# ribal-aladeeb/reinforcement-learning-2048

Measured on AMD Instinct MI355X. Metric: 2048 env steps/sec + DQN updates/sec at 64k parallel boards, 1→8 MI355X, higher is better.
Workload: dtype u8

## Files before the change

### reinforcement-learning-2048_amd/csrc/g2048_learn64.hip

```cpp
#include <hip/hip_runtime.h>
#include <math.h>
#include <stdint.h>
#include <stdlib.h>

#include "../../include/g2048.h"
#include "g2048_board.hpp"
#include "g2048_common.hpp"

namespace {

constexpr int NT = 256;
constexpr int S = 64;
constexpr int XS = 17;
constexpr int HS = 65;
constexpr int P_W1 = 0, P_B1 = 1024, P_W2 = 1088, P_B2 = 1344, P_N = 1348;
constexpr int SLAB = P_N + 4;
constexpr int MAX_SLABS = 256;

struct Net64 {
    double *w1, *b1, *w2, *b2;
};

struct alignas(16) Smem {
    double x[S * XS];
    double h[S * HS];
    double w2[2][4 * 64];
    double b1[2][64];
    double b2[2][4];
    double qa[S * 4];
    double qb[S * 4];
    double y[S];
    double dq[S];
    double loss[S];
    int act[S];
};

__device__ __forceinline__ int64_t sample_row(int64_t b, unsigned long long ep,
                                              unsigned long long count, uint32_t lo, uint32_t hi) {
    const uint4 u = g2048::philox10(
        make_uint4((uint32_t)b, (uint32_t)((uint64_t)b >> 32), (uint32_t)ep,
                   (uint32_t)(ep >> 32) | (g2048::DOMAIN_SAMPLE << 30)),
        lo, hi);
    return (int64_t)__umul64hi(((unsigned long long)u.y << 32) | u.x, count);
}

__device__ __forceinline__ void put_row(double* xr, uint4 v) {
    const uint32_t w[4] = {v.x, v.y, v.z, v.w};
#pragma unroll
    for (int k = 0; k < 4; ++k) {
        xr[4 * k + 0] = (double)(w[k] & 0xFFu);
        xr[4 * k + 1] = (double)((w[k] >> 8) & 0xFFu);
        xr[4 * k + 2] = (double)((w[k] >> 16) & 0xFFu);
        xr[4 * k + 3] = (double)(w[k] >> 24);
    }
}

__device__ __forceinline__ void forward(Smem& M, const double (&w1r)[16], int net, double* q) {
    const int t = threadIdx.x, j = t & 63, rq = t >> 6;
    const double bj = M.b1[net][j];
#pragma unroll 4
    for (int rr = 0; rr < 16; ++rr) {
        const int s = rq * 16 + rr;
        const double* xr = M.x + s * XS;
        double acc = 0.0;
#pragma unroll
        for (int k = 0; k < 16; ++k) acc = fma(w1r[k], xr[k], acc);
        const double pre = acc + bj;
        M.h[s * HS + j] = pre > 0.0 ? pre : 0.0;
    }
    __syncthreads();
    const int s = t >> 2, a = t & 3;
    const double* hr = M.h + s * HS;
    const double* w2 = M.w2[net] + a * 64;
    double acc = 0.0;
#pragma unroll 8
    for (int jj = 0; jj < 64; ++jj) acc = fma(w2[jj], hr[jj], acc);
    q[s * 4 + a] = acc + M.b2[net][a];
    __syncthreads();
}

struct UpdArgs64 {
    Net64 on, tg;
    const uint4 *s, *s2;
    const uint8_t *a, *d;
    const int32_t* r;
    const unsigned long long* count;
    const unsigned long long* step;
    const int64_t* idx_in;
    int64_t batch;
    uint32_t seed_lo, seed_hi;
    float gamma;
    int double_dqn;
    int64_t* idx_out;
    double* y_out;
    double* slab;
    unsigned long long* step_next;
};

typedef uint32_t u32x2 __attribute__((ext_vector_type(2)));
constexpr int AUX_SC1 = 16;
__device__ __forceinline__ __amdgpu_buffer_rsrc_t slab_rsrc(const double* base) {
    return __builtin_amdgcn_make_buffer_rsrc(const_cast<double*>(base), 0, 0x7FFFFFFF, 0x00020000);
}
template <bool COH>
__device__ __forceinline__ void slab_put(double* sl, int e, double v) {
    if constexpr (COH)
        __builtin_amdgcn_raw_buffer_store_b64(__builtin_bit_cast(u32x2, v), slab_rsrc(sl),
                                              (uint32_t)e * 8u, 0u, AUX_SC1);
    else
        sl[e] = v;
}

template <bool COH>
__device__ __forceinline__ void update_tiles64(const UpdArgs64& A) {
    __shared__ Smem M;
    const int t = threadIdx.x, j = t & 63, qd = t >> 6;
    const unsigned long long ep = A.idx_in ? 0ull : *A.step;
    const unsigned long long count = A.idx_in ? 0ull : *A.count;
    if (blockIdx.x == 0 && t == 0) *A.step_next = *A.step + 1ull;
    const Net64 nets[2] = {A.tg, A.on};
    double w1t[16], w1o[16];
#pragma unroll
    for (int k = 0; k < 16; ++k) {
        w1t[k] = A.tg.w1[j * 16 + k];
        w1o[k] = A.on.w1[j * 16 + k];
    }
    for (int i = t; i < 2 * 256; i += NT) M.w2[i >> 8][i & 255] = nets[i >> 8].w2[i & 255];
    if (t < 128) M.b1[t >> 6][t & 63] = nets[t >> 6].b1[t & 63];
    if (t < 8) M.b2[t >> 2][t & 3] = nets[t >> 2].b2[t & 3];
    double w2o[4];
#pragma unroll
    for (int a = 0; a < 4; ++a) w2o[a] = A.on.w2[a * 64 + j];
    double g_w1[4] = {0.0, 0.0, 0.0, 0.0}, g_b1 = 0.0, g_w2 = 0.0, g_b2 = 0.0, g_loss = 0.0;
    const int64_t ntiles = (A.batch + S - 1) / S;
    for (int64_t tile = blockIdx.x; tile < ntiles; tile += gridDim.x) {
        const int64_t b = tile * S + t;
        uint4 sv = make_uint4(0u, 0u, 0u, 0u);
        double rj = 0.0;
        float disc = 0.f;
        bool ok = false;
        __syncthreads();
        if (t < S) {
            uint4 s2v = make_uint4(0u, 0u, 0u, 0u);
            int aj = 0;
            ok = b < A.batch;
            if (ok) {
                const int64_t row =
                    A.idx_in ? A.idx_in[b] : sample_row(b, ep, count, A.seed_lo, A.seed_hi);
                A.idx_out[b] = row;
                s2v = A.s2[row];
                sv = A.s[row];
                aj = A.a[row];
                rj = (double)A.r[row];
                disc = (float)(1 - (int)A.d[row]) * A.gamma;
            }
            put_row(M.x + t * XS, s2v);
            M.act[t] = aj;
        }
        __syncthreads();
        forward(M, w1t, 0, M.qa);
        forward(M, w1o, 1, M.qb);
        if (t < S) {
            const double* qo = M.qb + t * 4;
            const double* qt = M.qa + t * 4;
            double next;
            if (A.double_dqn) {
                const uint32_t as = g2048::argmax4_torch(qo[0], qo[1], qo[2], qo[3]);
                next = qt[as];
            } else {
                next = g2048::qmax4_torch(qt[0], qt[1], qt[2], qt[3]);
            }
            double y;
            {
#pragma clang fp contract(off)
                y = rj + (double)disc * next;
            }
            M.y[t] = y;
            if (ok) A.y_out[b] = y;
            put_row(M.x + t * XS, sv);
        }
        __syncthreads();
        forward(M, w1o, 1, M.qb);
        if (t < S) {
            double dq = 0.0, l = 0.0;
            if (ok) {
#pragma clang fp contract(off)
                const double e = M.qb[t * 4 + M.act[t]] - M.y[t];
                dq = 2.0 * e;
                l = e * e;
            }
            M.dq[t] = dq;
            M.loss[t] = l;
        }
        __syncthreads();
        {
            double acc = 0.0, accb = 0.0;
            for (int s = 0; s < S; ++s) {
                if (M.act[s] == qd) {
                    acc = fma(M.dq[s], M.h[s * HS + j], acc);
                    accb += M.dq[s];
                }
            }
            g_w2 += acc;
            if (j == 0) g_b2 += accb;
        }
        if (t == 0) {
            double l = 0.0;
            for (int s = 0; s < S; ++s) l += M.loss[s];
            g_loss += l;
        }
        __syncthreads();
#pragma unroll 4
        for (int rr = 0; rr < 16; ++rr) {
            const int s = qd * 16 + rr;
            double& hv = M.h[s * HS + j];
            const double w = M.act[s] == 0 ? w2o[0] : M.act[s] == 1 ? w2o[1]
                           : M.act[s] == 2 ? w2o[2] : w2o[3];
            hv = hv > 0.0 ? M.dq[s] * w : 0.0;
        }
        __syncthreads();
        {
            double acc[4] = {0.0, 0.0, 0.0, 0.0}, accb = 0.0;
            for (int s = 0; s < S; ++s) {
                const double dh = M.h[s * HS + j];
                const double* xr = M.x + s * XS + 4 * qd;
#pragma unroll
                for (int i = 0; i < 4; ++i) acc[i] = fma(dh, xr[i], acc[i]);
                accb += dh;
            }
#pragma unroll
            for (int i = 0; i < 4; ++i) g_w1[i] += acc[i];
            if (qd == 0) g_b1 += accb;
        }
    }
    double* sl = A.slab + (int64_t)blockIdx.x * SLAB;
#pragma unroll
    for (int i = 0; i < 4; ++i) slab_put<COH>(sl, P_W1 + j * 16 + 4 * qd + i, g_w1[i]);
    if (qd == 0) slab_put<COH>(sl, P_B1 + j, g_b1);
    slab_put<COH>(sl, P_W2 + qd * 64 + j, g_w2);
    if (j == 0) slab_put<COH>(sl, P_B2 + qd, g_b2);
    if (t == 0) slab_put<COH>(sl, P_N, g_loss);
}

__global__ __launch_bounds__(NT) void k_dense64_update_f64(UpdArgs64 A) { update_tiles64<false>(A); }

constexpr int RW = 16;
static_assert(MAX_SLABS <= RW * 16, "reduction covers at most RW*16 slabs");

struct RedArgs64 {
    const double* slab;
    int nslab;
    double* grad;
    double* loss;
    const unsigned long long* step_next;
    unsigned long long* step;
    double* p[4];
    double* tp[4];
    unsigned long long sync_every;
    double* m;
    double* v;
    double lr, b1, b2, eps;
    int adam;
};

template <int NW, bool COH>
__device__ __forceinline__ void reduce_positions64(const RedArgs64& A, int chunk,
                                                   unsigned long long t, double (*part)[64]) {
    const int lane = threadIdx.x & 63, wave = threadIdx.x >> 6;
    const int pos = chunk * 64 + lane;
    const int k = pos < P_B1 ? 0 : pos < P_W2 ? 1 : pos < P_B2 ? 2 : 3;
    const int base[4] = {P_W1, P_B1, P_W2, P_B2};
    const bool adam = A.adam && wave == 0 && pos < P_N;
    double am = 0.0, av = 0.0, ap = 0.0;
    if (adam) {
        am = A.m[pos];
        av = A.v[pos];
        ap = A.p[k][pos - base[k]];
    }
    constexpr int PW = RW / NW;
    const bool okp = pos <= P_N;
    const int pc = okp ? pos : P_N;
    double v[PW][16];
#pragma unroll
    for (int i = 0; i < PW; ++i)
#pragma unroll
        for (int u = 0; u < 16; ++u) {
            const int g = wave + NW * i + RW * u;
            const bool ok = okp && g < A.nslab;
            const int64_t e = (int64_t)(g < A.nslab ? g : 0) * SLAB + pc;
            double x;
            if constexpr (COH)
                x = __builtin_bit_cast(double, __builtin_amdgcn_raw_buffer_load_b64(
                                                   slab_rsrc(A.slab), (uint32_t)(e * 8), 0u, AUX_SC1));
            else
                x = A.slab[e];
            v[i][u] = ok ? x : 0.0;
        }
#pragma unroll
    for (int i = 0; i < PW; ++i) {
        double r = 0.0;
#pragma unroll
        for (int u = 0; u < 16; ++u) r += v[i][u];
        part[wave + NW * i][lane] = r;
    }
    __syncthreads();
    if (wave == 0 && pos <= P_N) {
        double sum = part[0][lane];
        for (int j = 1; j < RW; ++j) sum += part[j][lane];
        if (pos == P_N) {
            if (A.loss) *A.loss = sum;
        } else {
            if (A.grad) A.grad[pos] = sum;
            if (adam) {
                const double np = g2048::adam64((double)t, A.lr, A.b1, A.b2, A.eps, sum, am, av, ap);
                A.m[pos] = am;
                A.v[pos] = av;
                A.p[k][pos - base[k]] = np;
                if (A.sync_every && t % A.sync_every == 0ull) A.tp[k][pos - base[k]] = np;
            }
        }
    }
}

constexpr int RCHUNKS = (P_N + 1 + 63) / 64;

__global__ __launch_bounds__(64 * RW) void k_dense64_reduce_f64(RedArgs64 A) {
    __shared__ double part[RW][64];
    reduce_positions64<RW, false>(A, blockIdx.x, A.adam ? *A.step_next : 0ull, part);
    if (A.step && blockIdx.x == 0 && threadIdx.x == 0) *A.step = *A.step_next;
}

struct Upd1Args64 {
    UpdArgs64 U;
    RedArgs64 R;
    unsigned int* arrive;
};

__global__ __launch_bounds__(NT) void k_dense64_update1_f64(Upd1Args64 A) {
    const unsigned long long t_next = *A.U.step + 1ull;
    update_tiles64<true>(A.U);
    __shared__ unsigned int s_arrival;
    __shared__ double part[RW][64];
    const unsigned grid = gridDim.x;
    __builtin_amdgcn_s_waitcnt(0);
    __syncthreads();
    if (threadIdx.x == 0)
        s_arrival = __hip_atomic_fetch_add(&A.arrive[0], 1u, __ATOMIC_RELAXED,
                                           __HIP_MEMORY_SCOPE_AGENT);
    __syncthreads();
    const unsigned a = s_arrival;
    const unsigned nred = grid < (unsigned)RCHUNKS ? grid : (unsigned)RCHUNKS;
    if (a >= grid) {
        if (threadIdx.x == 0) atomicAdd(&A.arrive[2], 1u);
        return;
    }
    if (a < grid - nred) return;
    const unsigned me = a - (grid - nred);
    if (threadIdx.x == 0) {
        unsigned it = 0;
        while (__hip_atomic_load(&A.arrive[0], __ATOMIC_RELAXED, __HIP_MEMORY_SCOPE_AGENT) < grid) {
            __builtin_amdgcn_s_sleep(1);
            if (++it == (1u << 24)) {
                atomicAdd(&A.arrive[2], 1u);
                break;
            }
        }
    }
    __syncthreads();
    for (unsigned c = me; c < (unsigned)RCHUNKS; c += nred) {
        reduce_positions64<NT / 64, true>(A.R, (int)c, t_next, part);
        __syncthreads();
    }
    if (threadIdx.x == 0) {
        if (me == 0 && A.R.step) *A.R.step = t_next;
        if (__hip_atomic_fetch_add(&A.arrive[1], 1u, __ATOMIC_RELAXED, __HIP_MEMORY_SCOPE_AGENT) ==
            nred - 1) {
            __hip_atomic_store(&A.arrive[0], 0u, __ATOMIC_RELAXED, __HIP_MEMORY_SCOPE_AGENT);
            __hip_atomic_store(&A.arrive[1], 0u, __ATOMIC_RELAXED, __HIP_MEMORY_SCOPE_AGENT);
        }
    }
}

}

extern "C" G2048_API int64_t g2048_dense64_update_f64_workspace(int64_t batch) {
    const int64_t tiles = (batch + S - 1) / S;
    const int64_t grid = tiles < MAX_SLABS ? tiles : MAX_SLABS;
    return grid * SLAB + 1 + 2;
}

extern "C" G2048_API int g2048_dense64_update_f64(
    const g2048_dense64_params_f64* online, const g2048_dense64_params_f64* target,
    g2048_replay* rb, const int64_t* idx_in, int64_t batch, uint64_t seed, uint64_t* step_dev,
    float gamma, int double_dqn, int64_t* idx_out, double* y_out, double* workspace,
    double* grad_out, double* loss_out, double* exp_avg, double* exp_avg_sq, double lr,
    double beta1, double beta2, double eps, uint64_t sync_every, void* stream) {
    if (!online || !target || !rb || batch <= 0 || !step_dev || !idx_out || !y_out || !workspace)
        return g2048_fail(G2048_EINVAL, "dense64_update_f64: NULL argument or batch <= 0");
    if (!online->w1 || !online->b1 || !online->w2 || !online->b2 || !target->w1 || !target->b1 ||
        !target->w2 || !target->b2)
        return g2048_fail(G2048_EINVAL, "dense64_update_f64: NULL parameter pointer");
    const bool adam = exp_avg && exp_avg_sq;
    if (!adam && !grad_out)
        return g2048_fail(G2048_EINVAL,
                          "dense64_update_f64: need exp_avg and exp_avg_sq (Adam) or grad_out");
    uint8_t *s = nullptr, *s2 = nullptr, *a = nullptr, *d = nullptr;
    int32_t* r = nullptr;
    uint64_t* count = nullptr;
    if (g2048_replay_views(rb, &s, &s2, &a, &r, &d, &count) != G2048_OK) return G2048_EINVAL;
    const int64_t tiles = (batch + S - 1) / S;
    const int grid = (int)(tiles < MAX_SLABS ? tiles : MAX_SLABS);
    UpdArgs64 U;
    U.on = Net64{online->w1, online->b1, online->w2, online->b2};
    U.tg = Net64{target->w1, target->b1, target->w2, target->b2};
    U.s = reinterpret_cast<const uint4*>(s);
    U.s2 = reinterpret_cast<const uint4*>(s2);
    U.a = a;
    U.d = d;
    U.r = r;
    U.count = reinterpret_cast<const unsigned long long*>(count);
    U.step = reinterpret_cast<const unsigned long long*>(step_dev);
    U.idx_in = idx_in;
    U.batch = batch;
    U.seed_lo = (uint32_t)seed;
    U.seed_hi = (uint32_t)(seed >> 32);
    U.gamma = gamma;
    U.double_dqn = double_dqn;
    U.idx_out = idx_out;
    U.y_out = y_out;
    U.slab = workspace;
    U.step_next = reinterpret_cast<unsigned long long*>(workspace + (int64_t)grid * SLAB);
    hipStream_t st = reinterpret_cast<hipStream_t>(stream);
    RedArgs64 R;
    R.slab = workspace;
    R.nslab = grid;
    R.grad = grad_out;
    R.loss = loss_out;
    R.step_next = U.step_next;
    R.step = reinterpret_cast<unsigned long long*>(step_dev);
    double* ps[4] = {online->w1, online->b1, online->w2, online->b2};
    double* ts[4] = {target->w1, target->b1, target->w2, target->b2};
    for (int k = 0; k < 4; ++k) {
        R.p[k] = ps[k];
        R.tp[k] = ts[k];
    }
    R.sync_every = adam ? sync_every : 0ull;
    R.m = exp_avg;
    R.v = exp_avg_sq;
    R.lr = lr;
    R.b1 = beta1;
    R.b2 = beta2;
    R.eps = eps;
    R.adam = adam ? 1 : 0;
    const char* one = getenv("G2048_DENSE64_ONE_LAUNCH");
    if (one && one[0] == '1') {
        Upd1Args64 A1;
        A1.U = U;
        A1.R = R;
        A1.arrive = reinterpret_cast<unsigned int*>(U.step_next + 1);
        hipLaunchKernelGGL(k_dense64_update1_f64, dim3(grid), dim3(NT), 0, st, A1);
    } else {
        hipLaunchKernelGGL(k_dense64_update_f64, dim3(grid), dim3(NT), 0, st, U);
        hipLaunchKernelGGL(k_dense64_reduce_f64, dim3(RCHUNKS), dim3(64 * RW), 0, st, R);
    }
    const hipError_t e = hipGetLastError();
    return e == hipSuccess ? G2048_OK
                           : g2048_fail(G2048_EHIP, "dense64_update_f64: %s", hipGetErrorString(e));
}
```

### reinforcement-learning-2048_amd/g2048/qnet.py

```python
from __future__ import annotations

import ctypes as C

import torch
from torch import nn

from . import _native as N
from .nets import Conv2048

_CONV_ORDER = ("0.weight", "0.bias", "2.weight", "2.bias", "5.weight", "5.bias", "7.weight",
               "7.bias")
_DENSE_ORDER = ("0.weight", "0.bias", "2.weight", "2.bias")


_DENSE_REF_ORDER = ("0.weight", "0.bias", "2.weight", "2.bias", "4.weight", "4.bias", "6.weight",
                    "6.bias")


def is_dense_ref(model) -> bool:
    dims = [(16, 512), (512, 512), (512, 256), (256, 4)]
    return (isinstance(model, nn.Sequential) and len(model) == 7
            and all(isinstance(model[2 * i], nn.Linear)
                    and (model[2 * i].in_features, model[2 * i].out_features) == d
                    for i, d in enumerate(dims))
            and all(isinstance(model[2 * i + 1], nn.ReLU) for i in range(3)))


class DenseForward:

    def __init__(self, model):
        if not is_dense_ref(model):
            raise TypeError("DenseForward needs the reference dense net (16-512-512-256-4)")
        dt = next(model.parameters()).dtype
        if dt not in (torch.float32, torch.float64):
            raise TypeError("DenseForward runs float32 or float64 nets")
        self.dtype = dt
        self.code = N.F32 if dt == torch.float32 else N.F64
        self._params = _tensors(model, _DENSE_REF_ORDER, dt)
        self.p = N.DenseNetParams(*[t.data_ptr() for t in self._params])

    def _out(self, n, device, out):
        if out is None:
            return torch.empty((n, 4), dtype=self.dtype, device=device)
        if out.shape != (n, 4) or out.dtype != self.dtype or not out.is_contiguous():
            raise ValueError(f"out must be a contiguous {self.dtype} [{n}, 4] tensor")
        return out

    def __call__(self, rows: torch.Tensor, idx: torch.Tensor | None = None,
                 out: torch.Tensor | None = None) -> torch.Tensor:
        if rows.dtype != torch.uint8 or rows.dim() != 2 or rows.shape[1] != 16 or not rows.is_contiguous():
            raise ValueError("rows must be a contiguous uint8 [*, 16] board tensor")
        if idx is not None and (idx.dtype != torch.int64 or not idx.is_contiguous()):
            raise ValueError("idx must be contiguous int64")
        n = rows.shape[0] if idx is None else idx.numel()
        out = self._out(n, rows.device, out)
        N.check(N.load().g2048_densenet_forward(C.byref(self.p), self.code, N.ptr(rows),
                                                N.ptr(idx), n, N.ptr(out),
                                                N.stream_of(rows.device)),
                "g2048_densenet_forward")
        return out

    def greedy(self, env, epsilon=0.0, eps_schedule=None, out: torch.Tensor | None = None):
        out = self._out(env.n, env.device, out)
        eps_ptr, eps_val, dec, mn = env.eps_args(epsilon, eps_schedule)
        N.check(N.load().g2048_densenet_forward_greedy(
            C.byref(self.p), self.code, env.handle, eps_ptr, eps_val, dec, mn, N.ptr(out),
            N.stream_of(env.device)), "g2048_densenet_forward_greedy")
        return out


def is_dense64(model) -> bool:
    return (isinstance(model, nn.Sequential) and len(model) == 3
            and isinstance(model[0], nn.Linear) and model[0].in_features == 16
            and model[0].out_features == 64 and isinstance(model[1], nn.ReLU)
            and isinstance(model[2], nn.Linear) and model[2].in_features == 64
            and model[2].out_features == 4)


def kind_of(model) -> str | None:
    if next(model.parameters()).dtype != torch.float32:
        return None
    if isinstance(model, Conv2048):
        return "conv"
    if is_dense64(model):
        return "dense64"
    return None


def kind64_of(model) -> str | None:
    if next(model.parameters()).dtype != torch.float64:
        return None
    if isinstance(model, Conv2048):
        return "conv"
    return "dense64" if is_dense64(model) else None


def update_kind(model) -> str | None:
    k = kind_of(model) or kind64_of(model)
    if k is None and is_dense_ref(model) and next(model.parameters()).dtype in (torch.float32,
                                                                                torch.float64):
        return "dense"
    return k


def _tensors(model, order, dtype=torch.float32):
    sd = dict(model.named_parameters())
    ts = [sd[k] for k in order]
    for t in ts:
        if t.dtype != dtype or not t.is_cuda or not t.is_contiguous():
            raise ValueError(f"fused Q-net kernels run {dtype} contiguous CUDA parameters")
    return ts


def net_params(model):
    k = kind_of(model)
    if k == "conv":
        return N.ConvNetParams(*[t.data_ptr() for t in _tensors(model, _CONV_ORDER)])
    if k == "dense64":
        return N.Dense64Params(*[t.data_ptr() for t in _tensors(model, _DENSE_ORDER)])
    raise TypeError("no fused kernel for this model (fp32 Conv2048 or dense 16-64-4 only)")


def _sym(model_or_kind, what):
    k = model_or_kind if isinstance(model_or_kind, str) else kind_of(model_or_kind)
    return getattr(N.load(), f"g2048_{'convnet' if k == 'conv' else 'dense64'}_{what}")


def conv_params(model: Conv2048) -> N.ConvNetParams:
    if not isinstance(model, Conv2048):
        raise TypeError("conv_params needs the reference conv net (g2048.nets.Conv2048)")
    return net_params(model)


def forward(model, rows: torch.Tensor, idx: torch.Tensor | None = None,
            out: torch.Tensor | None = None, params=None):
    if rows.dtype != torch.uint8 or rows.dim() != 2 or rows.shape[1] != 16 or not rows.is_contiguous():
        raise ValueError("rows must be a contiguous uint8 [*, 16] board tensor")
    n = rows.shape[0] if idx is None else idx.numel()
    if idx is not None and (idx.dtype != torch.int64 or not idx.is_contiguous()):
        raise ValueError("idx must be contiguous int64")
    if out is None:
        out = torch.empty((n, 4), dtype=torch.float32, device=rows.device)
    p = params if params is not None else net_params(model)
    N.check(_sym(model, "forward")(C.byref(p), N.ptr(rows), N.ptr(idx), n, N.ptr(out),
                                   N.stream_of(rows.device)), "fused forward")
    return out


conv_forward = forward


def forward_greedy(model, env, epsilon=0.0, eps_schedule=None, out: torch.Tensor | None = None,
                   params=None):
    if kind_of(model) != "conv":
        raise ValueError("forward_greedy: conv net only (the dense-64 step computes Q in-kernel)")
    if out is None:
        out = torch.empty((env.n, 4), dtype=torch.float32, device=env.device)
    if out.shape != (env.n, 4) or out.dtype != torch.float32 or not out.is_contiguous():
        raise ValueError(f"out must be a contiguous float32 [{env.n}, 4] tensor")
    eps_ptr, eps_val, dec, mn = env.eps_args(epsilon, eps_schedule)
    p = params if params is not None else net_params(model)
    N.check(N.load().g2048_convnet_forward_greedy(C.byref(p), env.handle, eps_ptr, eps_val, dec,
                                                  mn, N.ptr(out), N.stream_of(env.device)),
            "g2048_convnet_forward_greedy")
    return out


CONV64_FWD_WORKSPACE = 53248


class ConvForward64:

    def __init__(self, model):
        if kind64_of(model) != "conv":
            raise TypeError("ConvForward64 needs an fp64 Conv2048")
        self.p = N.ConvNetParams(*[t.data_ptr() for t in
                                   _tensors(model, _CONV_ORDER, torch.float64)])
        self.ws = torch.empty(CONV64_FWD_WORKSPACE, dtype=torch.float64,
                              device=next(model.parameters()).device)

    def __call__(self, rows: torch.Tensor, idx: torch.Tensor | None = None,
                 out: torch.Tensor | None = None) -> torch.Tensor:
        if rows.dtype != torch.uint8 or rows.dim() != 2 or rows.shape[1] != 16 or not rows.is_contiguous():
            raise ValueError("rows must be a contiguous uint8 [*, 16] board tensor")
        if idx is not None and (idx.dtype != torch.int64 or not idx.is_contiguous()):
            raise ValueError("idx must be contiguous int64")
        n = rows.shape[0] if idx is None else idx.numel()
        if out is None:
            out = torch.empty((n, 4), dtype=torch.float64, device=rows.device)
        N.check(N.load().g2048_convnet_forward_f64(C.byref(self.p), N.ptr(rows), N.ptr(idx), n,
                                                   N.ptr(out), N.ptr(self.ws),
                                                   N.stream_of(rows.device)),
                "g2048_convnet_forward_f64")
        return out

    def greedy(self, env, epsilon=0.0, eps_schedule=None, out: torch.Tensor | None = None):
        if out is None:
            out = torch.empty((env.n, 4), dtype=torch.float64, device=env.device)
        if out.shape != (env.n, 4) or out.dtype != torch.float64 or not out.is_contiguous():
            raise ValueError(f"out must be a contiguous float64 [{env.n}, 4] tensor")
        eps_ptr, eps_val, dec, mn = env.eps_args(epsilon, eps_schedule)
        N.check(N.load().g2048_convnet_forward_greedy_f64(
            C.byref(self.p), env.handle, eps_ptr, eps_val, dec, mn, N.ptr(out), N.ptr(self.ws),
            N.stream_of(env.device)), "g2048_convnet_forward_greedy_f64")
        return out


class TrainGrad:

    def __init__(self, model, batch: int, adam=None):
        self.kind = kind_of(model)
        self.params = net_params(model)
        self.batch = int(batch)
        self.n_params = sum(p.numel() for p in model.parameters())
        if adam is not None and self.kind != "conv":
            raise TypeError("the Adam-folded reduction exists for the conv net only")
        self.adam = adam
        self._tparams = None
        if adam is not None and adam.sync_every:
            tps = list(adam._target)
            if len(tps) != 8:
                raise ValueError("the attached target must be the conv net's 8 tensors")
            self._tparams = N.ConvNetParams(*[t.data_ptr() for t in tps])
        dev = next(model.parameters()).device
        n = _sym(self.kind, "train_workspace")(self.batch)
        self.workspace = torch.empty(n, dtype=torch.float32, device=dev)

    def __call__(self, rows: torch.Tensor, actions: torch.Tensor, idx: torch.Tensor,
                 y: torch.Tensor, grad_out: torch.Tensor | None, loss_out: torch.Tensor | None = None,
                 step: torch.Tensor | None = None):
        if idx.numel() != self.batch or y.numel() != self.batch:
            raise ValueError("idx / y must have `batch` elements")
        if y.dtype != torch.float32 or (grad_out is not None and (
                grad_out.dtype != torch.float32 or grad_out.numel() != self.n_params)):
            raise ValueError(f"y and grad_out must be float32; grad_out has {self.n_params} elements")
        a = self.adam
        if a is None:
            if grad_out is None:
                raise ValueError("without Adam state the gradient needs a grad_out buffer")
            N.check(_sym(self.kind, "train_grad")(
                C.byref(self.params), N.ptr(rows), N.ptr(actions), N.ptr(idx), N.ptr(y), self.batch,
                N.ptr(self.workspace), N.ptr(grad_out), N.ptr(loss_out), N.ptr(step),
                N.stream_of(rows.device)), "fused train_grad")
            return
        if step is None:
            raise ValueError("the Adam-folded update needs the device step counter")
        tp = C.byref(self._tparams) if self._tparams is not None else None
        N.check(N.load().g2048_convnet_train_adam(
            C.byref(self.params), N.ptr(rows), N.ptr(actions), N.ptr(idx), N.ptr(y), self.batch,
            N.ptr(self.workspace), N.ptr(grad_out), N.ptr(loss_out), N.ptr(step),
            N.ptr(a.exp_avg), N.ptr(a.exp_avg_sq), a.lr, a.betas[0], a.betas[1], a.eps, tp,
            int(a.sync_every) if self._tparams is not None else 0, N.stream_of(rows.device)),
            "g2048_convnet_train_adam")


ConvTrainGrad = TrainGrad


class ConvUpdate:

    def __init__(self, model, target, batch: int, adam=None):
        if kind_of(model) != "conv" or kind_of(target) != "conv":
            raise TypeError("ConvUpdate needs the conv net for online and target")
        self.on, self.tg = net_params(model), net_params(target)
        self.batch = int(batch)
        self.adam = adam
        dev = next(model.parameters()).device
        n = N.load().g2048_convnet_train_workspace(self.batch)
        self.workspace = torch.empty(n, dtype=torch.float32, device=dev)

    def __call__(self, replay, idx_out, y_out, step_dev, gamma=0.8, double_dqn=True, seed=0,
                 idx_in=None, grad_out=None, loss_out=None):
        if idx_out.numel() != self.batch or y_out.numel() != self.batch:
            raise ValueError("idx_out / y_out must have `batch` elements")
        if self.adam is None and grad_out is None:
            raise ValueError("without Adam state the gradient needs a grad_out buffer")
        a = self.adam
        m, v = (a.exp_avg, a.exp_avg_sq) if a is not None else (None, None)
        lr, b1, b2, eps = (a.lr, a.betas[0], a.betas[1], a.eps) if a is not None else (0, 0, 0, 0)
        N.check(N.load().g2048_convnet_update(
            C.byref(self.on), C.byref(self.tg), replay.handle, N.ptr(idx_in), self.batch,
            int(seed), N.ptr(step_dev), float(gamma), int(bool(double_dqn)), N.ptr(idx_out),
            N.ptr(y_out), N.ptr(self.workspace), N.ptr(grad_out), N.ptr(loss_out), N.ptr(m),
            N.ptr(v), float(lr), float(b1), float(b2), float(eps),
            int(a.sync_every) if a is not None else 0, N.stream_of(y_out.device)),
            "g2048_convnet_update")


class Adam64:

    def __init__(self, params, lr: float = 1e-2, betas=(0.9, 0.999), eps: float = 1e-8):
        self.params = list(params)
        self.lr, self.betas, self.eps = float(lr), (float(betas[0]), float(betas[1])), float(eps)
        n = sum(p.numel() for p in self.params)
        dev = self.params[0].device
        self.exp_avg = torch.zeros(n, dtype=torch.float64, device=dev)
        self.exp_avg_sq = torch.zeros(n, dtype=torch.float64, device=dev)
        self.sync_every = 0

        self._ptrs = (C.c_void_p * len(self.params))(*[p.data_ptr() for p in self.params])
        self._numel = (C.c_int64 * len(self.params))(*[p.numel() for p in self.params])
        self._tptrs = None

    def attach_target(self, target_params, sync_every: int) -> None:
        self._target = list(target_params)
        self._tptrs = (C.c_void_p * len(self._target))(*[t.data_ptr() for t in self._target])
        self.sync_every = int(sync_every)

    def reset_state(self):
        self.exp_avg.zero_()
        self.exp_avg_sq.zero_()

    def step(self, grad_flat: torch.Tensor, step_counter: torch.Tensor, grad_scale: float = 1.0):
        lib = N.load()
        args = (self._ptrs, self._numel, len(self.params), N.ptr(grad_flat), N.ptr(self.exp_avg),
                N.ptr(self.exp_avg_sq), N.ptr(step_counter), self.lr, self.betas[0], self.betas[1],
                self.eps, self._tptrs, self.sync_every if self._tptrs is not None else 0)
        if grad_scale == 1.0:
            N.check(lib.g2048_adam_step_sync_f64(*args, N.stream_of(grad_flat.device)),
                    "g2048_adam_step_sync_f64")
        else:
            N.check(lib.g2048_adam_step_scaled_f64(*args, float(grad_scale),
                                                   N.stream_of(grad_flat.device)),
                    "g2048_adam_step_scaled_f64")


class Dense64Update64:

    def __init__(self, model, target, batch: int, adam: Adam64 | None = None):
        if kind64_of(model) != "dense64" or kind64_of(target) != "dense64":
            raise TypeError("Dense64Update64 needs fp64 dense 16-64-4 online and target nets")
        self.on = N.Dense64Params(*[t.data_ptr() for t in
                                    _tensors(model, _DENSE_ORDER, torch.float64)])
        self.tg = N.Dense64Params(*[t.data_ptr() for t in
                                    _tensors(target, _DENSE_ORDER, torch.float64)])
        self.batch = int(batch)
        self.adam = adam
        dev = next(model.parameters()).device
        n = N.load().g2048_dense64_update_f64_workspace(self.batch)
        self.workspace = torch.zeros(n, dtype=torch.float64, device=dev)
        self._grid = min((self.batch + 63) // 64, 256)

    def sync_errors(self) -> int:
        return int(self.workspace[self._grid * 1352 + 1:].view(torch.int32)[2])

    def __call__(self, replay, idx_out, y_out, step_dev, gamma=0.8, double_dqn=True, seed=0,
                 idx_in=None, grad_out=None, loss_out=None):
        if idx_out.numel() != self.batch or y_out.numel() != self.batch:
            raise ValueError("idx_out / y_out must have `batch` elements")
        if y_out.dtype != torch.float64:
            raise TypeError("y_out must be float64")
        if self.adam is None and grad_out is None:
            raise ValueError("without Adam state the gradient needs a grad_out buffer")
        a = self.adam
        m, v = (a.exp_avg, a.exp_avg_sq) if a is not None else (None, None)
        lr, b1, b2, eps = (a.lr, a.betas[0], a.betas[1], a.eps) if a is not None else (0, 0, 0, 0)
        N.check(N.load().g2048_dense64_update_f64(
            C.byref(self.on), C.byref(self.tg), replay.handle, N.ptr(idx_in), self.batch,
            int(seed), N.ptr(step_dev), float(gamma), int(bool(double_dqn)), N.ptr(idx_out),
            N.ptr(y_out), N.ptr(self.workspace), N.ptr(grad_out), N.ptr(loss_out), N.ptr(m),
            N.ptr(v), float(lr), float(b1), float(b2), float(eps),
            int(a.sync_every) if a is not None else 0, N.stream_of(y_out.device)),
            "g2048_dense64_update_f64")


class ConvUpdate64:

    def __init__(self, model, target, batch: int, adam: Adam64 | None = None):
        if kind64_of(model) != "conv" or kind64_of(target) != "conv":
            raise TypeError("ConvUpdate64 needs fp64 Conv2048 online and target nets")
        self._params = (_tensors(model, _CONV_ORDER, torch.float64)
                        + _tensors(target, _CONV_ORDER, torch.float64))
        self.on = N.ConvNetParams(*[t.data_ptr() for t in self._params[:8]])
        self.tg = N.ConvNetParams(*[t.data_ptr() for t in self._params[8:]])
        self.batch = int(batch)
        self.adam = adam
        dev = next(model.parameters()).device
        n = N.load().g2048_convnet_update_f64_workspace(self.batch)
        self.workspace = torch.empty(n, dtype=torch.float64, device=dev)
        self._packed_at = None
        self.ensure_packed()

    def _versions(self):
        return tuple(t._version for t in self._params)

    def ensure_packed(self, force: bool = False) -> bool:
        v = self._versions()
        if not force and v == self._packed_at:
            return False
        N.check(N.load().g2048_convnet_pack_f64(C.byref(self.on), C.byref(self.tg),
                                                N.ptr(self.workspace),
                                                N.stream_of(self.workspace.device)),
                "g2048_convnet_pack_f64")
        self._packed_at = v
        return True

    def __call__(self, replay, idx_out, y_out, step_dev, gamma=0.8, double_dqn=True, seed=0,
                 idx_in=None, grad_out=None, loss_out=None):
        if idx_out.numel() != self.batch or y_out.numel() != self.batch:
            raise ValueError("idx_out / y_out must have `batch` elements")
        if y_out.dtype != torch.float64:
            raise TypeError("y_out must be float64")
        if self.adam is None and grad_out is None:
            raise ValueError("without Adam state the gradient needs a grad_out buffer")
        if not torch.cuda.is_current_stream_capturing():
            self.ensure_packed()
        a = self.adam
        m, v = (a.exp_avg, a.exp_avg_sq) if a is not None else (None, None)
        lr, b1, b2, eps = (a.lr, a.betas[0], a.betas[1], a.eps) if a is not None else (0, 0, 0, 0)
        N.check(N.load().g2048_convnet_update_f64(
            C.byref(self.on), C.byref(self.tg), replay.handle, N.ptr(idx_in), self.batch,
            int(seed), N.ptr(step_dev), float(gamma), int(bool(double_dqn)), N.ptr(idx_out),
            N.ptr(y_out), N.ptr(self.workspace), N.ptr(grad_out), N.ptr(loss_out), N.ptr(m),
            N.ptr(v), float(lr), float(b1), float(b2), float(eps),
            int(a.sync_every) if a is not None else 0, N.stream_of(y_out.device)),
            "g2048_convnet_update_f64")


class DenseRefUpdate:

    def __init__(self, model, target, batch: int, adam=None):
        if not (is_dense_ref(model) and is_dense_ref(target)):
            raise TypeError("DenseRefUpdate needs the reference dense net for online and target")
        dt = next(model.parameters()).dtype
        if dt not in (torch.float32, torch.float64):
            raise TypeError("DenseRefUpdate runs float32 or float64 nets")
        self.dtype = dt
        self.code = N.F32 if dt == torch.float32 else N.F64
        self._params = (_tensors(model, _DENSE_REF_ORDER, dt)
                        + _tensors(target, _DENSE_REF_ORDER, dt))
        self.on = N.DenseNetParams(*[t.data_ptr() for t in self._params[:8]])
        self.tg = N.DenseNetParams(*[t.data_ptr() for t in self._params[8:]])
        self.batch = int(batch)
        self.adam = adam
        dev = next(model.parameters()).device
        n = N.load().g2048_densenet_update_workspace(self.batch, self.code)
        self.workspace = torch.empty(n, dtype=dt, device=dev)

    def __call__(self, replay, idx_out, y_out, step_dev, gamma=0.8, double_dqn=True, seed=0,
                 idx_in=None, grad_out=None, loss_out=None):
        if idx_out.numel() != self.batch or y_out.numel() != self.batch:
            raise ValueError("idx_out / y_out must have `batch` elements")
        if y_out.dtype != self.dtype:
            raise TypeError(f"y_out must be {self.dtype}")
        if self.adam is None and grad_out is None:
            raise ValueError("without Adam state the gradient needs a grad_out buffer")
        a = self.adam
        m, v = (a.exp_avg, a.exp_avg_sq) if a is not None else (None, None)
        lr, b1, b2, eps = (a.lr, a.betas[0], a.betas[1], a.eps) if a is not None else (0, 0, 0, 0)
        N.check(N.load().g2048_densenet_update(
            C.byref(self.on), C.byref(self.tg), self.code, replay.handle, N.ptr(idx_in),
            self.batch, int(seed), N.ptr(step_dev), float(gamma), int(bool(double_dqn)),
            N.ptr(idx_out), N.ptr(y_out), N.ptr(self.workspace), N.ptr(grad_out),
            N.ptr(loss_out), N.ptr(m), N.ptr(v), float(lr), float(b1), float(b2), float(eps),
            int(a.sync_every) if a is not None else 0, N.stream_of(y_out.device)),
            "g2048_densenet_update")


class Dense64Update:

    def __init__(self, model, target, batch: int, adam=None):
        if kind_of(model) != "dense64" or kind_of(target) != "dense64":
            raise TypeError("Dense64Update needs fp32 dense 16-64-4 online and target nets")
        self.on, self.tg = net_params(model), net_params(target)
        self.batch = int(batch)
        self.adam = adam
        dev = next(model.parameters()).device
        n = N.load().g2048_dense64_update_workspace(self.batch)
        self.workspace = torch.zeros(n, dtype=torch.float32, device=dev)
        self._grid = min((self.batch + 31) // 32, 256)

    def sync_errors(self) -> int:
        tail = self.workspace[self._grid * 1352 + 2:].view(torch.int32)
        return int(tail[2])

    def __call__(self, replay, idx_out, y_out, step_dev, gamma=0.8, double_dqn=True, seed=0,
                 idx_in=None, grad_out=None, loss_out=None):
        if idx_out.numel() != self.batch or y_out.numel() != self.batch:
            raise ValueError("idx_out / y_out must have `batch` elements")
        if self.adam is None and grad_out is None:
            raise ValueError("without Adam state the gradient needs a grad_out buffer")
        a = self.adam
        m, v = (a.exp_avg, a.exp_avg_sq) if a is not None else (None, None)
        lr, b1, b2, eps = (a.lr, a.betas[0], a.betas[1], a.eps) if a is not None else (0, 0, 0, 0)
        N.check(N.load().g2048_dense64_update(
            C.byref(self.on), C.byref(self.tg), replay.handle, N.ptr(idx_in), self.batch,
            int(seed), N.ptr(step_dev), float(gamma), int(bool(double_dqn)), N.ptr(idx_out),
            N.ptr(y_out), N.ptr(self.workspace), N.ptr(grad_out), N.ptr(loss_out), N.ptr(m),
            N.ptr(v), float(lr), float(b1), float(b2), float(eps),
            int(a.sync_every) if a is not None else 0, N.stream_of(y_out.device)),
            "g2048_dense64_update")


def targets(kind: str, online, target, replay, batch: int, idx_out: torch.Tensor,
            y_out: torch.Tensor, gamma: float = 0.8, double_dqn: bool = True, seed: int = 0,
            epoch: torch.Tensor | None = None, idx_in: torch.Tensor | None = None):
    if idx_in is None and epoch is None:
        raise ValueError("need idx_in or a device epoch counter")
    N.check(_sym(kind, "targets")(
        C.byref(online), C.byref(target), replay.handle, N.ptr(idx_in), int(batch), int(seed),
        N.ptr(epoch), float(gamma), int(bool(double_dqn)), N.ptr(idx_out), N.ptr(y_out),
        N.stream_of(y_out.device)), "fused targets")
    return idx_out, y_out


def conv_targets(online, target, replay, batch, idx_out, y_out, gamma=0.8, double_dqn=True,
                 seed=0, epoch=None, idx_in=None):
    return targets("conv", online, target, replay, batch, idx_out, y_out, gamma, double_dqn,
                   seed, epoch, idx_in)
```

Measured before the change: 170.7 billion.

## Use f64 MFMA for dense64 DQN update forward and W1 gradient

Rewrites the fp64 dense 16-64-4 update kernel so that the first-layer forward pass and the W1 gradient run on MFMA f64 16x16x4 instructions instead of scalar FMA loops. Tile size drops from 64 to 32 samples, and the second layer is split across 8 threads per sample with two partial sums. Replay rows are now gathered one word per thread, and shared-memory strides are padded. The smaller tile doubles the grid cap per batch and changes the FP summation order, so results may not match the old ordering bit for bit. The Python grid and sync_errors offsets are updated to match.

```diff
diff --git a/reinforcement-learning-2048_amd/csrc/g2048_learn64.hip b/reinforcement-learning-2048_amd/csrc/g2048_learn64.hip
--- a/reinforcement-learning-2048_amd/csrc/g2048_learn64.hip
+++ b/reinforcement-learning-2048_amd/csrc/g2048_learn64.hip
@@ -10,9 +10,8 @@
 namespace {
 
 constexpr int NT = 256;
-constexpr int S = 64;
-constexpr int XS = 17;
-constexpr int HS = 65;
+constexpr int S = 32;
+constexpr int XS = 18, HS = 68, W2S = 68;
 constexpr int P_W1 = 0, P_B1 = 1024, P_W2 = 1088, P_B2 = 1344, P_N = 1348;
 constexpr int SLAB = P_N + 4;
 constexpr int MAX_SLABS = 256;
@@ -24,16 +23,17 @@
 struct alignas(16) Smem {
     double x[S * XS];
     double h[S * HS];
-    double w2[2][4 * 64];
+    double w2[2][4 * W2S];
     double b1[2][64];
     double b2[2][4];
-    double qa[S * 4];
-    double qb[S * 4];
-    double y[S];
+    double qa[S * 8];
+    double qb[S * 8];
     double dq[S];
     double loss[S];
     int act[S];
 };
+
+typedef double d4 __attribute__((ext_vector_type(4)));
 
 __device__ __forceinline__ int64_t sample_row(int64_t b, unsigned long long ep,
                                               unsigned long long count, uint32_t lo, uint32_t hi) {
@@ -44,38 +44,69 @@
     return (int64_t)__umul64hi(((unsigned long long)u.y << 32) | u.x, count);
 }
 
-__device__ __forceinline__ void put_row(double* xr, uint4 v) {
-    const uint32_t w[4] = {v.x, v.y, v.z, v.w};
-#pragma unroll
-    for (int k = 0; k < 4; ++k) {
-        xr[4 * k + 0] = (double)(w[k] & 0xFFu);
-        xr[4 * k + 1] = (double)((w[k] >> 8) & 0xFFu);
-        xr[4 * k + 2] = (double)((w[k] >> 16) & 0xFFu);
-        xr[4 * k + 3] = (double)(w[k] >> 24);
-    }
-}
-
-__device__ __forceinline__ void forward(Smem& M, const double (&w1r)[16], int net, double* q) {
-    const int t = threadIdx.x, j = t & 63, rq = t >> 6;
-    const double bj = M.b1[net][j];
-#pragma unroll 4
-    for (int rr = 0; rr < 16; ++rr) {
-        const int s = rq * 16 + rr;
-        const double* xr = M.x + s * XS;
-        double acc = 0.0;
-#pragma unroll
-        for (int k = 0; k < 16; ++k) acc = fma(w1r[k], xr[k], acc);
-        const double pre = acc + bj;
-        M.h[s * HS + j] = pre > 0.0 ? pre : 0.0;
-    }
-    __syncthreads();
-    const int s = t >> 2, a = t & 3;
-    const double* hr = M.h + s * HS;
-    const double* w2 = M.w2[net] + a * 64;
-    double acc = 0.0;
-#pragma unroll 8
-    for (int jj = 0; jj < 64; ++jj) acc = fma(w2[jj], hr[jj], acc);
-    q[s * 4 + a] = acc + M.b2[net][a];
+__device__ __forceinline__ void put_word(double* dst, uint32_t v) {
+    double2* d = reinterpret_cast<double2*>(dst);
+    d[0] = make_double2((double)(v & 0xFFu), (double)((v >> 8) & 0xFFu));
+    d[1] = make_double2((double)((v >> 16) & 0xFFu), (double)(v >> 24));
+}
+
+struct W1Lane {
+    double v[4];
+};
+__device__ __forceinline__ W1Lane w1_lane(const double* w1) {
+    const int lane = threadIdx.x & 63, wave = threadIdx.x >> 6;
+    const double2* p = reinterpret_cast<const double2*>(w1 + (16 * wave + (lane & 15)) * 16 +
+                                                        4 * (lane >> 4));
+    const double2 a = p[0], b = p[1];
+    return W1Lane{{a.x, a.y, b.x, b.y}};
+}
+
+__device__ __forceinline__ void forward(Smem& M, const W1Lane& w1v, int net, double* q) {
+    const int t = threadIdx.x;
+    {
+        const int lane = t & 63, wave = t >> 6, lk = lane >> 4, lr = lane & 15;
+        const int j = 16 * wave + lr;
+        const double bj = M.b1[net][j];
+#pragma unroll
+        for (int mb = 0; mb < S / 16; ++mb) {
+            const double2* xr =
+                reinterpret_cast<const double2*>(M.x + (16 * mb + lr) * XS + 4 * lk);
+            const double2 x01 = xr[0], x23 = xr[1];
+            d4 acc = {0.0, 0.0, 0.0, 0.0};
+            acc = __builtin_amdgcn_mfma_f64_16x16x4f64(x01.x, w1v.v[0], acc, 0, 0, 0);
+            acc = __builtin_amdgcn_mfma_f64_16x16x4f64(x01.y, w1v.v[1], acc, 0, 0, 0);
+            acc = __builtin_amdgcn_mfma_f64_16x16x4f64(x23.x, w1v.v[2], acc, 0, 0, 0);
+            acc = __builtin_amdgcn_mfma_f64_16x16x4f64(x23.y, w1v.v[3], acc, 0, 0, 0);
+#pragma unroll
+            for (int r = 0; r < 4; ++r) {
+                const double pre = acc[r] + bj;
+                M.h[(16 * mb + 4 * r + lk) * HS + j] = pre > 0.0 ? pre : 0.0;
+            }
+        }
+    }
+    __syncthreads();
+    {
+        const int s = t >> 3, a = (t >> 1) & 3, half = t & 1;
+        const double2* hr = reinterpret_cast<const double2*>(M.h + s * HS) + half;
+        const double2* wr = reinterpret_cast<const double2*>(M.w2[net] + a * W2S) + half;
+        double e = half ? 0.0 : M.b2[net][a], o = 0.0;
+#pragma unroll
+        for (int u0 = 0; u0 < 16; u0 += 8) {
+            double2 hv[8], wv[8];
+#pragma unroll
+            for (int u = 0; u < 8; ++u) {
+                hv[u] = hr[2 * (u0 + u)];
+                wv[u] = wr[2 * (u0 + u)];
+            }
+            __builtin_amdgcn_sched_barrier(0);
+#pragma unroll
+            for (int u = 0; u < 8; ++u) {
+                e = fma(wv[u].x, hv[u].x, e);
+                o = fma(wv[u].y, hv[u].y, o);
+            }
+        }
+        q[t] = e + o;
+    }
     __syncthreads();
 }
 
@@ -114,132 +145,145 @@
 template <bool COH>
 __device__ __forceinline__ void update_tiles64(const UpdArgs64& A) {
     __shared__ Smem M;
-    const int t = threadIdx.x, j = t & 63, qd = t >> 6;
+    const int t = threadIdx.x, lane = t & 63, wave = t >> 6, lk = lane >> 4, lr = lane & 15;
     const unsigned long long ep = A.idx_in ? 0ull : *A.step;
     const unsigned long long count = A.idx_in ? 0ull : *A.count;
     if (blockIdx.x == 0 && t == 0) *A.step_next = *A.step + 1ull;
-    const Net64 nets[2] = {A.tg, A.on};
-    double w1t[16], w1o[16];
-#pragma unroll
-    for (int k = 0; k < 16; ++k) {
-        w1t[k] = A.tg.w1[j * 16 + k];
-        w1o[k] = A.on.w1[j * 16 + k];
-    }
-    for (int i = t; i < 2 * 256; i += NT) M.w2[i >> 8][i & 255] = nets[i >> 8].w2[i & 255];
-    if (t < 128) M.b1[t >> 6][t & 63] = nets[t >> 6].b1[t & 63];
-    if (t < 8) M.b2[t >> 2][t & 3] = nets[t >> 2].b2[t & 3];
-    double w2o[4];
-#pragma unroll
-    for (int a = 0; a < 4; ++a) w2o[a] = A.on.w2[a * 64 + j];
-    double g_w1[4] = {0.0, 0.0, 0.0, 0.0}, g_b1 = 0.0, g_w2 = 0.0, g_b2 = 0.0, g_loss = 0.0;
+    const W1Lane w1t = w1_lane(A.tg.w1), w1o = w1_lane(A.on.w1);
+    M.w2[0][wave * W2S + lane] = A.tg.w2[t];
+    M.w2[1][wave * W2S + lane] = A.on.w2[t];
+    if (t < 128) M.b1[t >> 6][t & 63] = (t < 64 ? A.tg.b1 : A.on.b1)[t & 63];
+    if (t < 8) M.b2[t >> 2][t & 3] = (t < 4 ? A.tg.b2 : A.on.b2)[t & 3];
+    d4 g_w1a = {0.0, 0.0, 0.0, 0.0};
+    d4 g_w1b = {0.0, 0.0, 0.0, 0.0};
+    double g_b1 = 0.0, g_w2 = 0.0, g_b2 = 0.0, g_loss = 0.0;
     const int64_t ntiles = (A.batch + S - 1) / S;
+    const int sl = t >> 2, w = t & 3;
+    const bool own = t < 4 * S && w == 0;
+    const uint32_t* s2w32 = reinterpret_cast<const uint32_t*>(A.s2);
+    const uint32_t* sw32 = reinterpret_cast<const uint32_t*>(A.s);
     for (int64_t tile = blockIdx.x; tile < ntiles; tile += gridDim.x) {
-        const int64_t b = tile * S + t;
-        uint4 sv = make_uint4(0u, 0u, 0u, 0u);
-        double rj = 0.0;
-        float disc = 0.f;
-        bool ok = false;
-        __syncthreads();
-        if (t < S) {
-            uint4 s2v = make_uint4(0u, 0u, 0u, 0u);
-            int aj = 0;
-            ok = b < A.batch;
-            if (ok) {
-                const int64_t row =
-                    A.idx_in ? A.idx_in[b] : sample_row(b, ep, count, A.seed_lo, A.seed_hi);
+        const int64_t b = tile * S + sl;
+        const bool ok = t < 4 * S && b < A.batch;
+        uint32_t s2w = 0u, sw = 0u;
+        int32_t rw = 0;
+        uint8_t dj = 1, aw = 0;
+        if (ok) {
+            const int64_t row =
+                A.idx_in ? A.idx_in[b] : sample_row(b, ep, count, A.seed_lo, A.seed_hi);
+            s2w = s2w32[row * 4 + w];
+            sw = sw32[row * 4 + w];
+            if (w == 0) {
                 A.idx_out[b] = row;
-                s2v = A.s2[row];
-                sv = A.s[row];
-                aj = A.a[row];
-                rj = (double)A.r[row];
-                disc = (float)(1 - (int)A.d[row]) * A.gamma;
-            }
-            put_row(M.x + t * XS, s2v);
-            M.act[t] = aj;
+                aw = A.a[row];
+                rw = A.r[row];
+                dj = A.d[row];
+            }
+        }
+        __syncthreads();
+        const int aj = aw;
+        if (t < 4 * S) {
+            put_word(M.x + sl * XS + 4 * w, s2w);
+            if (w == 0) M.act[sl] = aj;
         }
         __syncthreads();
         forward(M, w1t, 0, M.qa);
         forward(M, w1o, 1, M.qb);
-        if (t < S) {
-            const double* qo = M.qb + t * 4;
-            const double* qt = M.qa + t * 4;
+        double y = 0.0;
+        if (own) {
+            const double rj = (double)rw;
+            const float disc = (float)(1 - (int)dj) * A.gamma;
+            const double* qo = M.qb + sl * 8;
+            const double* qt = M.qa + sl * 8;
             double next;
             if (A.double_dqn) {
-                const uint32_t as = g2048::argmax4_torch(qo[0], qo[1], qo[2], qo[3]);
-                next = qt[as];
+                const uint32_t as = g2048::argmax4_torch(qo[0] + qo[1], qo[2] + qo[3],
+                                                         qo[4] + qo[5], qo[6] + qo[7]);
+                next = qt[2 * as] + qt[2 * as + 1];
             } else {
-                next = g2048::qmax4_torch(qt[0], qt[1], qt[2], qt[3]);
-            }
-            double y;
+                next = g2048::qmax4_torch(qt[0] + qt[1], qt[2] + qt[3], qt[4] + qt[5],
+                                          qt[6] + qt[7]);
+            }
             {
 #pragma clang fp contract(off)
                 y = rj + (double)disc * next;
             }
-            M.y[t] = y;
             if (ok) A.y_out[b] = y;
-            put_row(M.x + t * XS, sv);
-        }
+        }
+        if (t < 4 * S) put_word(M.x + sl * XS + 4 * w, sw);
         __syncthreads();
         forward(M, w1o, 1, M.qb);
-        if (t < S) {
-            double dq = 0.0, l = 0.0;
+        if (own) {
+            double dq = 0.0;
             if (ok) {
 #pragma clang fp contract(off)
-                const double e = M.qb[t * 4 + M.act[t]] - M.y[t];
+                const double e = (M.qb[sl * 8 + 2 * aj] + M.qb[sl * 8 + 2 * aj + 1]) - y;
                 dq = 2.0 * e;
-                l = e * e;
-            }
-            M.dq[t] = dq;
-            M.loss[t] = l;
+                g_loss += e * e;
+            }
+            M.dq[sl] = dq;
         }
         __syncthreads();
         {
-            double acc = 0.0, accb = 0.0;
-            for (int s = 0; s < S; ++s) {
-                if (M.act[s] == qd) {
-                    acc = fma(M.dq[s], M.h[s * HS + j], acc);
-                    accb += M.dq[s];
+            double e = 0.0, o = 0.0, eb = 0.0, ob = 0.0;
+#pragma unroll 8
+            for (int s = 0; s < S; s += 2) {
+                const double g0 = M.act[s] == wave ? M.dq[s] : 0.0;
+                const double g1 = M.act[s + 1] == wave ? M.dq[s + 1] : 0.0;
+                e = fma(g0, M.h[s * HS + lane], e);
+                o = fma(g1, M.h[(s + 1) * HS + lane], o);
+                eb += g0;
+                ob += g1;
+            }
+            g_w2 += e + o;
+            if (lane == 0) g_b2 += eb + ob;
+        }
+        __syncthreads();
+        {
+            constexpr int SPT = S / 4;
+#pragma unroll
+            for (int ss = 0; ss < SPT; ++ss) {
+                const int s = wave * SPT + ss;
+                const double hv = M.h[s * HS + lane];
+                M.h[s * HS + lane] = hv > 0.0 ? M.dq[s] * M.w2[1][M.act[s] * W2S + lane] : 0.0;
+            }
+        }
+        __syncthreads();
+        {
+            const double* hc = M.h + 16 * wave + lr;
+            const double* xc = M.x + lr;
+#pragma unroll
+            for (int st = 0; st < S / 4; st += 2) {
+                g_w1a = __builtin_amdgcn_mfma_f64_16x16x4f64(
+                    hc[(4 * st + lk) * HS], xc[(4 * st + lk) * XS], g_w1a, 0, 0, 0);
+                g_w1b = __builtin_amdgcn_mfma_f64_16x16x4f64(
+                    hc[(4 * st + 4 + lk) * HS], xc[(4 * st + 4 + lk) * XS], g_w1b, 0, 0, 0);
+            }
+            if (t < 64) {
+                double e = 0.0, o = 0.0;
+#pragma unroll 8
+                for (int s = 0; s < S; s += 2) {
+                    e += M.h[s * HS + t];
+                    o += M.h[(s + 1) * HS + t];
                 }
-            }
-            g_w2 += acc;
-            if (j == 0) g_b2 += accb;
-        }
-        if (t == 0) {
-            double l = 0.0;
-            for (int s = 0; s < S; ++s) l += M.loss[s];
-            g_loss += l;
-        }
-        __syncthreads();
-#pragma unroll 4
-        for (int rr = 0; rr < 16; ++rr) {
-            const int s = qd * 16 + rr;
-            double& hv = M.h[s * HS + j];
-            const double w = M.act[s] == 0 ? w2o[0] : M.act[s] == 1 ? w2o[1]
-                           : M.act[s] == 2 ? w2o[2] : w2o[3];
-            hv = hv > 0.0 ? M.dq[s] * w : 0.0;
-        }
-        __syncthreads();
-        {
-            double acc[4] = {0.0, 0.0, 0.0, 0.0}, accb = 0.0;
-            for (int s = 0; s < S; ++s) {
-                const double dh = M.h[s * HS + j];
-                const double* xr = M.x + s * XS + 4 * qd;
-#pragma unroll
-                for (int i = 0; i < 4; ++i) acc[i] = fma(dh, xr[i], acc[i]);
-                accb += dh;
-            }
-#pragma unroll
-            for (int i = 0; i < 4; ++i) g_w1[i] += acc[i];
-            if (qd == 0) g_b1 += accb;
-        }
-    }
-    double* sl = A.slab + (int64_t)blockIdx.x * SLAB;
-#pragma unroll
-    for (int i = 0; i < 4; ++i) slab_put<COH>(sl, P_W1 + j * 16 + 4 * qd + i, g_w1[i]);
-    if (qd == 0) slab_put<COH>(sl, P_B1 + j, g_b1);
-    slab_put<COH>(sl, P_W2 + qd * 64 + j, g_w2);
-    if (j == 0) slab_put<COH>(sl, P_B2 + qd, g_b2);
-    if (t == 0) slab_put<COH>(sl, P_N, g_loss);
+                g_b1 += e + o;
+            }
+        }
+    }
+    double* slab = A.slab + (int64_t)blockIdx.x * SLAB;
+#pragma unroll
+    for (int r = 0; r < 4; ++r)
+        slab_put<COH>(slab, P_W1 + (16 * wave + 4 * r + lk) * 16 + lr, g_w1a[r] + g_w1b[r]);
+    if (t < 64) slab_put<COH>(slab, P_B1 + t, g_b1);
+    slab_put<COH>(slab, P_W2 + t, g_w2);
+    if (lane == 0) slab_put<COH>(slab, P_B2 + wave, g_b2);
+    if (own) M.loss[sl] = g_loss;
+    __syncthreads();
+    if (t == 0) {
+        double l = 0.0;
+        for (int s = 0; s < S; ++s) l += M.loss[s];
+        slab_put<COH>(slab, P_N, l);
+    }
 }
 
 __global__ __launch_bounds__(NT) void k_dense64_update_f64(UpdArgs64 A) { update_tiles64<false>(A); }
diff --git a/reinforcement-learning-2048_amd/g2048/qnet.py b/reinforcement-learning-2048_amd/g2048/qnet.py
--- a/reinforcement-learning-2048_amd/g2048/qnet.py
+++ b/reinforcement-learning-2048_amd/g2048/qnet.py
@@ -339,10 +339,10 @@
         dev = next(model.parameters()).device
         n = N.load().g2048_dense64_update_f64_workspace(self.batch)
         self.workspace = torch.zeros(n, dtype=torch.float64, device=dev)
-        self._grid = min((self.batch + 63) // 64, 256)
+        self._grid = min((self.batch + 31) // 32, 256)
 
     def sync_errors(self) -> int:
-        return int(self.workspace[self._grid * 1352 + 1:].view(torch.int32)[2])
+        return int(self.workspace[-2:].view(torch.int32)[2])
 
     def __call__(self, replay, idx_out, y_out, step_dev, gamma=0.8, double_dqn=True, seed=0,
                  idx_in=None, grad_out=None, loss_out=None):
@@ -471,8 +471,7 @@
         self._grid = min((self.batch + 31) // 32, 256)
 
     def sync_errors(self) -> int:
-        tail = self.workspace[self._grid * 1352 + 2:].view(torch.int32)
-        return int(tail[2])
+        return int(self.workspace[-4:].view(torch.int32)[2])
 
     def __call__(self, replay, idx_out, y_out, step_dev, gamma=0.8, double_dqn=True, seed=0,
                  idx_in=None, grad_out=None, loss_out=None):
```

After: 171.0 billion, median of 4. About the same (+0.2%).
